# lcrekko/lq_mpc

Measured on AMD Instinct MI355X. Metric: MPC QP-steps/sec (batched systems) at n_x=4,n_u=2,N=10; 1/2/4/8 GPU, higher is better.
Workload: dtype f64

## Files before the change

lq_mpc_amd/csrc/lqmpc_r16_body.h:

```cpp
#pragma once
#include "lqmpc_wg_linalg.h"
#include "lqmpc_r16_setup.h"

namespace lqmpc {

using wg::ldsd;
using wg::ldsi;
using wg::rowb;
using wg::fmac_rowb;
using wg::fmac_rowb_self;
using wg::fmac_rowb4;
using wg::fmac_rowb_self4;
using wg::fmac_rowb_self2;
using wg::fmac_rowb_self3;
using wg::fmac_rowb_lanes4;
using wg::fmac_rowb_lanes4x2;
using wg::dpp_settle;

#ifdef LQMPC_R16_PROF
__device__ long long g_r16_prof[32];
#define RPROF(k) do { const long long now_ = clock64(); if (threadIdx.x == 0 && blockIdx.x == PROFBLK) g_r16_prof[k] += now_ - prof_t; if (k < 7) prof_ph[k] += now_ - prof_t; prof_t = clock64(); } while (0)
#define RPROF_START long long prof_t = clock64()
#define RPROF_ADD(k, v) do { if (threadIdx.x == 0) atomicAdd((unsigned long long *)&g_r16_prof[k], (unsigned long long)(v)); } while (0)
#ifndef PROFBLK
#define PROFBLK 0
#endif
#else
#define RPROF(k) do { } while (0)
#define RPROF_START do { } while (0)
#define RPROF_ADD(k, v) do { } while (0)
#endif

typedef unsigned long long mask_t;

template <int NX, int NU, int N, int LPI = 16, bool PACKED = false>
struct R16 {
    static constexpr int n = N * NU;
    static constexpr int RB = (n + LPI - 1) / LPI;
    static constexpr int IPW = 64 / LPI;
    static constexpr int CS = 4 * (((n + 1) / 2 + 3) / 4);
    static constexpr int LDW = n + 1;
    static constexpr int PK = PACKED ? n * (n + 1) / 2 : n * LDW;
    static constexpr int VEC = LPI * RB;
    static constexpr int oP = 0, oW = PK, oR = 2 * PK, oX = oR + VEC, oY = oX + VEC, oL = oY + VEC;
    static constexpr int oC = oL + CS / 2;
    static constexpr int CN0 = 3 * NX * NX + NU * NU + NX * NU;
    static constexpr int CN1 = (NX > NU ? NX : NU) * (2 * NX + 2 * NU);
    static constexpr int CN = CN0 > CN1 ? CN0 : CN1;
    static constexpr int SETUP = n * NX;
    static constexpr int oG = 0;
    static constexpr int END = oC + CN + (CN & 1);
    static constexpr int oD = (END > SETUP) ? END : SETUP;
    static constexpr int INST = oD + 2;
    static constexpr int MAXIT = 12;
    static_assert(LPI == 16 || LPI == 64, "a DPP row or the whole wavefront");
    static_assert((n + 1) / 2 <= CS && n <= 64, "the smaller side must fit the gathered system");
};


template <int LPI>
__device__ __forceinline__ mask_t iballot(bool c, int q)
{
    if constexpr (LPI == 16) return (__ballot(c) >> (16 * q)) & 0xFFFFull;
    else return __ballot(c);
}
template <int LPI>
__device__ __forceinline__ double ibcast(double x, int k)
{
    if constexpr (LPI == 16) return rowb(x, k);
    else return wg::rdlane(x, k);
}
template <int LPI>
__device__ __forceinline__ void ifmac(double &acc, double x, double y, int k)
{
    if constexpr (LPI == 16) fmac_rowb(acc, x, y, k);
    else acc = __builtin_fma(wg::rdlane(x, k), y, acc);
}
template <int LPI>
__device__ __forceinline__ void ifmac_self(double &acc, double y, int k)
{
    if constexpr (LPI == 16) fmac_rowb_self(acc, y, k);
    else acc = __builtin_fma(wg::rdlane(acc, k), y, acc);
}
template <int LPI>
__device__ __forceinline__ void ifmac4(double *acc, const double *x, double y, int k)
{
    if constexpr (LPI == 16) fmac_rowb4(acc[0], acc[1], acc[2], acc[3], x[0], x[1], x[2], x[3], y, k);
    else {
#pragma unroll
        for (int e = 0; e < 4; ++e) acc[e] = __builtin_fma(wg::rdlane(x[e], k), y, acc[e]);
    }
}
template <int LPI>
__device__ __forceinline__ void ifmac_self4(double *acc, double y, int k)
{
    if constexpr (LPI == 16) fmac_rowb_self4(acc[0], acc[1], acc[2], acc[3], y, k);
    else {
#pragma unroll
        for (int e = 0; e < 4; ++e) acc[e] = __builtin_fma(wg::rdlane(acc[e], k), y, acc[e]);
    }
}
template <int LPI, int K, int CS>
__device__ __forceinline__ void ifmac_self_tail(double (&S)[CS], double &rhs, double g)
{
    constexpr int r = K % 4;
    if constexpr (LPI == 16) {
        if constexpr (r == 0) fmac_rowb_self4(S[K + 1], S[K + 2], S[K + 3], rhs, g, K);
        else if constexpr (r == 1) fmac_rowb_self3(S[K + 1], S[K + 2], rhs, g, K);
        else if constexpr (r == 2) fmac_rowb_self2(S[K + 1], rhs, g, K);
        else fmac_rowb_self(rhs, g, K);
    } else {
#pragma unroll
        for (int j = K + 1; j < 4 * (K / 4) + 4; ++j) S[j] = __builtin_fma(wg::rdlane(S[j], K), g, S[j]);
        rhs = __builtin_fma(wg::rdlane(rhs, K), g, rhs);
    }
}
template <int LPI>
__device__ __forceinline__ void isettle(double &x)
{
    if constexpr (LPI == 16) dpp_settle(x);
}
__device__ __forceinline__ int rowb_i(int x, int c)
{
    switch (c) {
#define LQMPC_X(C) case C: return __builtin_amdgcn_update_dpp(0, x, 0x150 + C, 0xF, 0xF, true);
        LQMPC_ROWB_CASES(LQMPC_X)
#undef LQMPC_X
    }
    return x;
}
__device__ __forceinline__ unsigned row_or(unsigned x)
{
    x |= (unsigned)__builtin_amdgcn_update_dpp(0, (int)x, 0x128, 0xF, 0xF, false);
    x |= (unsigned)__builtin_amdgcn_update_dpp(0, (int)x, 0x124, 0xF, 0xF, false);
    x |= (unsigned)__builtin_amdgcn_update_dpp(0, (int)x, 0x122, 0xF, 0xF, false);
    x |= (unsigned)__builtin_amdgcn_update_dpp(0, (int)x, 0x121, 0xF, 0xF, false);
    return x;
}
__device__ __forceinline__ unsigned row_umax(unsigned x)
{
    x = max(x, (unsigned)__builtin_amdgcn_update_dpp(0, (int)x, 0x128, 0xF, 0xF, false));
    x = max(x, (unsigned)__builtin_amdgcn_update_dpp(0, (int)x, 0x124, 0xF, 0xF, false));
    x = max(x, (unsigned)__builtin_amdgcn_update_dpp(0, (int)x, 0x122, 0xF, 0xF, false));
    x = max(x, (unsigned)__builtin_amdgcn_update_dpp(0, (int)x, 0x121, 0xF, 0xF, false));
    return x;
}

template <int CNT, typename F>
__device__ __forceinline__ void static_for(F &&f) { sfor<0, CNT>(f); }

template <int NX, int NU, int N, int MODE, int LPI = 16, int OCC = 1>
__device__ __forceinline__ void r16_body(const KParams &p, double *lds_raw, long long slot0, long long slot_end)
{
    constexpr bool PACKED = (OCC == 2);
    using C = R16<NX, NU, N, LPI, PACKED>;
    constexpr int CS = C::CS;
    constexpr int n = C::n, RB = C::RB, LDW = C::LDW;
    constexpr int REC = NX * NX + NX * NU + NX;
    const int lane = threadIdx.x, q = lane / LPI, i = lane % LPI;
    ldsd *L = (ldsd *)lds_raw + q * C::INST;
    ldsd *Pp = L + C::oP, *Wp = L + C::oW, *rL = L + C::oR, *xL = L + C::oX, *yL = L + C::oY;
    ldsi *list = (ldsi *)(L + C::oL);
    const long long Bsz = p.Bsz;
    const long long b_raw = slot0 + q;
    const bool valid = b_raw < slot_end;
    const long long slot = valid ? b_raw : slot_end - 1;
    const long long b = p.perm ? (long long)p.perm[slot] : slot;
    const double *sh = p.sh;
    const mask_t nmask = (n == 64) ? ~0ull : ((1ull << n) - 1ull);

    int rw[RB], tri[RB];
    bool vrow[RB];
#pragma unroll
    for (int s = 0; s < RB; ++s) {
        rw[s] = i + LPI * s;
        tri[s] = rw[s] * (rw[s] + 1) / 2;
        vrow[s] = rw[s] < n;
    }

    auto ad = [&](int r, int tr, int j) -> int { if constexpr (PACKED) return (j <= r) ? tr + j : j * (j + 1) / 2 + r; else return r * LDW + j; };
    auto ad2 = [&](int a, int b2) -> int {
        if constexpr (PACKED) { const int hi = a > b2 ? a : b2, lo = a > b2 ? b2 : a; return hi * (hi + 1) / 2 + lo; }
        else return a * LDW + b2;
    };

    double G[RB][NX], vr[RB];
    constexpr bool LAZY_P = (LPI == 64);
    bool P_ready = !LAZY_P;
#ifdef LQMPC_NO_ROLL
    constexpr bool ROLL = false;
#else
    constexpr bool ROLL = LPI == 16 && N * ((NX + 3) / 4) <= 12 && MODE != MODE_MAXVN;
#endif
    unsigned cold32[2] = {0u, 0u};
    bool cold_armed = false;
#ifdef LQMPC_R16_PROF
    const long long prof_t0 = clock64();
    int prof_wit = 0, prof_slow = 0, prof_fast = 0;
    long long prof_slowt = 0;
    long long prof_ph[8] = {0, 0, 0, 0, 0, 0, 0, 0};
#endif
    {
        RPROF_START;
        long long bg = b;
        ldsd *Lg = L;
        if constexpr (LPI == 16) {
            const int gq = (lane >> 2) & 3;
            const long long sraw = slot0 + gq, sl = sraw < slot_end ? sraw : slot_end - 1;
            bg = p.perm ? (long long)p.perm[sl] : sl;
            Lg = (ldsd *)lds_raw + gq * C::INST;
        }
        r16_setup_mfma<NX, NU, N, LPI, PACKED, RB, ROLL>(setup_args(p), bg, Lg, L, C::oW, C::oG, C::oD, G, roll_args(p), cold32[0], cold32[1]);
        if constexpr (!LAZY_P) r16_build_P<NX, NU, N, LPI, PACKED>(setup_args(p), bg, Lg, C::oP, C::oD);
        RPROF(5);
        const bool has_lin = p.has_lin != 0;
#pragma unroll
        for (int s = 0; s < RB; ++s) vr[s] = 0.0;
        if (has_lin) {
            if (p.has_ref) {
                double qr[RB];
#pragma unroll
                for (int s = 0; s < RB; ++s) qr[s] = 0.0;
                double lam[NX], A2[NX][NX], B2[NX][NU];
#pragma unroll
                for (int a = 0; a < NX; ++a) {
                    lam[a] = 0.0;
#pragma unroll
                    for (int c = 0; c < NX; ++c) A2[a][c] = p.rec ? p.rec[b * REC + a * NX + c] : p.A[(long long)(a * NX + c) * Bsz + b];
#pragma unroll
                    for (int k = 0; k < NU; ++k) B2[a][k] = p.rec ? p.rec[b * REC + NX * NX + a * NU + k] : p.B[(long long)(a * NU + k) * Bsz + b];
                }
#pragma unroll 1
                for (int r = N - 1; r >= 0; --r) {
                    const int oQ = (r < N - 1) ? p.so.Q : p.so.P;
                    double l2[NX];
#pragma unroll
                    for (int a = 0; a < NX; ++a) {
                        double t = 0.0;
#pragma unroll
                        for (int c = 0; c < NX; ++c) t = __builtin_fma(sh[oQ + a * NX + c], -sh[p.so.xref + c * N + r], t);
#pragma unroll
                        for (int c = 0; c < NX; ++c) t = __builtin_fma(A2[c][a], lam[c], t);
                        l2[a] = t;
                    }
#pragma unroll
                    for (int a = 0; a < NX; ++a) lam[a] = l2[a];
#pragma unroll
                    for (int s = 0; s < RB; ++s) {
                        const int ui = rw[s] % NU;
                        double t = 0.0;
#pragma unroll
                        for (int k = 0; k < NU; ++k) {
                            double tk = 0.0;
#pragma unroll
                            for (int a = 0; a < NX; ++a) tk = __builtin_fma(B2[a][k], lam[a], tk);
#pragma unroll
                            for (int j = 0; j < NU; ++j) tk = __builtin_fma(-sh[p.so.R + k * NU + j], sh[p.so.uref + j * N + r], tk);
                            t = (ui == k) ? tk : t;
                        }
                        qr[s] = (vrow[s] && rw[s] / NU == r) ? 2.0 * t : qr[s];
                    }
                }
#pragma unroll
                for (int s = 0; s < RB; ++s) xL[rw[s]] = qr[s];
                __syncthreads();
#pragma unroll
                for (int s = 0; s < RB; ++s) {
                    double t = 0.0;
                    const int mr = vrow[s] ? rw[s] : 0, mt = vrow[s] ? tri[s] : 0;
#pragma unroll
                    for (int j = 0; j < n; ++j) t = __builtin_fma(Wp[ad(mr, mt, j)], xL[j], t);
                    vr[s] = -t;
                }
                __syncthreads();
            }
#pragma unroll
            for (int s = 0; s < RB; ++s) {
                const int k = rw[s] % NU;
                vr[s] = vrow[s] ? vr[s] - 0.5 * (sh[p.so.ub + k] + sh[p.so.lb + k]) : 0.0;
            }
        }
        if constexpr (LAZY_P && MODE != MODE_MAXVN) {
            mask_t out = 0;
#pragma unroll
            for (int s = 0; s < RB; ++s) {
                double acc = vr[s];
#pragma unroll
                for (int a = 0; a < NX; ++a) acc = __builtin_fma(G[s][a], p.rec ? p.rec[b * REC + NX * NX + NX * NU + a] : p.x0[(long long)a * Bsz + b], acc);
                const int k = rw[s] % NU;
                out |= iballot<LPI>(vrow[s] && !(fabs(acc) <= 0.5 * (sh[p.so.ub + k] - sh[p.so.lb + k])), q) << (LPI * s);
            }
            if (__ballot(2 * __popcll(out) > n) != 0ull) {
                r16_build_P<NX, NU, N, LPI, PACKED>(setup_args(p), bg, Lg, C::oP, C::oD);
                P_ready = true;
            }
        }
        RPROF(6);
    }
    RPROF_START;
    RPROF_ADD(13, clock64() - prof_t0);

    long long bq = b;
    asm volatile("" : "+v"(bq));
    double h[RB], ctr[RB];
#pragma unroll
    for (int s = 0; s < RB; ++s) {
        const int k = rw[s] % NU;
        h[s] = vrow[s] ? 0.5 * (sh[p.so.ub + k] - sh[p.so.lb + k]) : 1.0;
        ctr[s] = vrow[s] ? 0.5 * (sh[p.so.ub + k] + sh[p.so.lb + k]) : 0.0;
    }
    double Qm[NX][NX], Rm[NU][NU];
    ldsd *cQ = L + C::oC, *cR = cQ + NX * NX;
    if constexpr (MODE == MODE_ROLLOUT) {
    } else if constexpr (OCC == 2) {
        if (i == 0) {
#pragma unroll
            for (int a = 0; a < NX; ++a) {
#pragma unroll
                for (int c = 0; c < NX; ++c) {
                    cQ[a * NX + c] = sh[p.so.Q + a * NX + c];
                }
            }
#pragma unroll
            for (int k = 0; k < NU; ++k)
#pragma unroll
                for (int j = 0; j < NU; ++j) cR[k * NU + j] = sh[p.so.R + k * NU + j];
        }
        __syncthreads();
    } else {
#pragma unroll
        for (int a = 0; a < NX; ++a) {
#pragma unroll
            for (int c = 0; c < NX; ++c) Qm[a][c] = sh[p.so.Q + a * NX + c];
        }
#pragma unroll
        for (int k = 0; k < NU; ++k)
#pragma unroll
            for (int j = 0; j < NU; ++j) Rm[k][j] = sh[p.so.R + k * NU + j];
    }
    auto Qv = [&](int a, int c) -> double { if constexpr (OCC == 2) return cQ[a * NX + c]; else return Qm[a][c]; };
    auto Rv = [&](int k, int j) -> double { if constexpr (OCC == 2) return cR[k * NU + j]; else return Rm[k][j]; };
    const bool writer = valid && i == 0;
    mask_t pL = 0, pU = 0;
    int iters = 0, status = 0;
    auto qp = [&](const double (&x)[NX], double (&v)[RB]) {
        double vu[RB];
        mask_t cl = 0, cu = 0;
        bool bad = false;
#pragma unroll
        for (int s = 0; s < RB; ++s) {
            double acc = vr[s];
#pragma unroll
            for (int a = 0; a < NX; ++a) acc = __builtin_fma(G[s][a], x[a], acc);
            vu[s] = acc; v[s] = acc;
            cl |= iballot<LPI>(vrow[s] && acc < -h[s], q) << (LPI * s);
            cu |= iballot<LPI>(vrow[s] && acc > h[s], q) << (LPI * s);
            bad = bad || (vrow[s] && !(fabs(acc) < 1e300));
        }
        const bool rowbad = iballot<LPI>(bad, q) != 0;
        bool busy = ((cl | cu) != 0) && !rowbad;
        mask_t mL = 0, mU = 0;
        if (busy) {
            if (p.warm_start && (pL | pU) != 0) {
                const mask_t top = nmask & ~(nmask >> NU);
                mL = (pL >> NU) | (pL & top);
                mU = (pU >> NU) | (pU & top);
            } else if (ROLL && cold_armed && (cold32[0] | cold32[1]) != 0u) {
                mL = cold32[0]; mU = cold32[1];
            } else {
                mL = cl; mU = cu;
            }
        }
        cold_armed = false;
        bool failed = false;
        int it = 0;
        bool need_P = false;
#pragma unroll 1
        do {
        if (LAZY_P && need_P) {
            long long bg = bq;
            ldsd *Lg = L;
            if constexpr (LPI == 16) {
                const int gq = (lane >> 2) & 3;
                const long long sraw = slot0 + gq, sl = sraw < slot_end ? sraw : slot_end - 1;
                bg = p.perm ? (long long)p.perm[sl] : sl;
                Lg = (ldsd *)lds_raw + gq * C::INST;
            }
            r16_build_P<NX, NU, N, LPI, PACKED>(setup_args(p), bg, Lg, C::oP, C::oD);
            P_ready = true;
            need_P = false;
        }
        if (__ballot(busy) != 0ull) {
#pragma unroll 1
            for (; it < p.r16_maxit; ++it) {
#ifdef LQMPC_R16_PROF
                const long long prof_it0 = clock64();
#endif
                const mask_t mA = mL | mU;
                const int m = __popcll(mA);
                constexpr int DUAL_MAX = (LPI == 16 && n >= 16) ? (n / 2 + 2 < CS ? n / 2 + 2 : CS) : n / 2;
                const bool dual = m <= DUAL_MAX;
                const mask_t mC = busy ? (dual ? mA : (~mA & nmask)) : 0ull;
                const int c = __popcll(mC);
                int cw;
                if constexpr (LPI == 16)
                    cw = max(max(__builtin_amdgcn_readlane(c, 0), __builtin_amdgcn_readlane(c, 16)),
                             max(__builtin_amdgcn_readlane(c, 32), __builtin_amdgcn_readlane(c, 48)));
                else cw = __builtin_amdgcn_readfirstlane(c);
                const bool any_primal = __ballot(busy && !dual) != 0ull;
                if (LAZY_P && any_primal && !P_ready) { need_P = true; break; }
                if constexpr (LPI == 16) {
                    if (!any_primal) {
                        const unsigned mC32 = (unsigned)mC, mL32 = (unsigned)mL, mA32 = (unsigned)mA;
#pragma unroll
                        for (int s = 0; s < RB; ++s) {
                            const unsigned bit = 1u << rw[s];
                            const bool on = vrow[s] && (mC32 & bit);
                            const int rk = __popc(mC32 & (bit - 1u));
                            const double sg = (mL32 & bit) ? -1.0 : 1.0;
                            list[on ? rk : (C::oD - C::oL) * 2] = rw[s];
                            rL[on ? rk : C::oD - C::oR] = __builtin_fma(-sg, h[s], vu[s]);
                        }
                        __syncthreads();
                        const bool mine = i < c;
                        const int la = mine ? list[i] : 0;
                        double rhs = mine ? rL[i] : 0.0;
                        const int tla = PACKED ? la * (la + 1) / 2 : la * LDW;
                        auto widx = [&](int ra, int ta, int lb, int tlb) -> int {
                            if constexpr (PACKED) return max(ta, tlb) + min(ra, lb);
                            else return ta + lb;
                        };
                        double S[CS];
                        static_for<CS / 4>([&](auto bgc) {
                            constexpr int bg = decltype(bgc)::value;
#pragma unroll
                            for (int bb = 4 * bg; bb < 4 * bg + 4; ++bb) S[bb] = (bb == i) ? 1.0 : 0.0;
                            if (4 * bg < cw) {
                                static_for<4>([&](auto bc) {
                                    constexpr int bb = 4 * bg + decltype(bc)::value;
                                    const int lb = rowb_i(la, bb), tlb = PACKED ? rowb_i(tla, bb) : 0;
                                    const double val = Wp[widx(la, tla, lb, tlb)];
                                    S[bb] = mine ? val : S[bb];
                                });
                            }
                        });
                        bool ok = true;
                        static_for<CS>([&](auto kc) {
                            constexpr int k = decltype(kc)::value;
                            if (k < cw) {
                                isettle<LPI>(S[k]);
                                const double d = ibcast<LPI>(S[k], k);
                                ok = ok && (d > 0.0);
                                const double inv = frcp1(d);
                                const double g = (i == k) ? (inv - 1.0) : -S[k] * inv;
#pragma unroll
                                for (int jg = 0; jg < CS / 4; ++jg)
                                    if (4 * jg > k && 4 * jg < cw) ifmac_self4<LPI>(&S[4 * jg], g, k);
                                ifmac_self_tail<LPI, k>(S, rhs, g);
                            }
                        });
                        const bool rowfail = iballot<LPI>(!ok, q) != 0;
                        double tt[RB];
#pragma unroll
                        for (int s = 0; s < RB; ++s) tt[s] = 0.0;
                        const int trow[2] = {PACKED ? tri[0] : rw[0] * LDW, RB > 1 ? (PACKED ? tri[RB - 1] : rw[RB - 1] * LDW) : 0};
                        static_for<CS / 4>([&](auto kgc) {
                            constexpr int kg = decltype(kgc)::value;
                            if (4 * kg < cw) {
                                double wv[4][RB];
                                static_for<4>([&](auto kc) {
                                    constexpr int kk = decltype(kc)::value;
                                    const int lk = rowb_i(la, 4 * kg + kk), tlk = PACKED ? rowb_i(tla, 4 * kg + kk) : 0;
#pragma unroll
                                    for (int s = 0; s < RB; ++s) wv[kk][s] = Wp[vrow[s] ? widx(rw[s], trow[s], lk, tlk) : 0];
                                });
                                if constexpr (RB == 2) fmac_rowb_lanes4x2(tt[0], tt[1], rhs, wv[0][0], wv[0][1], wv[1][0], wv[1][1], wv[2][0], wv[2][1], wv[3][0], wv[3][1], 4 * kg);
                                else if constexpr (RB == 1) fmac_rowb_lanes4(tt[0], rhs, wv[0][0], wv[1][0], wv[2][0], wv[3][0], 4 * kg);
                                else {
                                    static_for<4>([&](auto kc) {
                                        constexpr int kk = decltype(kc)::value;
#pragma unroll
                                        for (int s = 0; s < RB; ++s) fmac_rowb(tt[s], rhs, wv[kk][s], 4 * kg + kk);
                                    });
                                }
                            }
                        });
                        const unsigned lhi = (unsigned)__double2hiint(rhs) & 0x7fffffffu;
                        const double tol = 1e-10 * __hiloint2double((int)row_umax(mine ? lhi : 0u), 0);
                        const bool isL = (mL32 >> la) & 1u;
                        const unsigned keepL = (mine && isL && rhs <= tol) ? (1u << la) : 0u;
                        const unsigned keepU = (mine && !isL && rhs >= -tol) ? (1u << la) : 0u;
                        unsigned nL32 = row_or(keepL), nU32 = row_or(keepU);
                        bool nf = false;
#pragma unroll
                        for (int s = 0; s < RB; ++s) {
                            const unsigned bit = 1u << rw[s];
                            const bool act = vrow[s] && (mA32 & bit);
                            const double sg = (mL32 & bit) ? -1.0 : 1.0;
                            const double nv = act ? sg * h[s] : vu[s] - tt[s];
                            v[s] = busy ? nv : v[s];
                            const bool fr = vrow[s] && !act;
                            nL32 |= (unsigned)(iballot<LPI>(fr && v[s] < -h[s] * (1.0 + 1e-12), q) << (LPI * s));
                            nU32 |= (unsigned)(iballot<LPI>(fr && v[s] > h[s] * (1.0 + 1e-12), q) << (LPI * s));
                            nf = nf || (vrow[s] && !(fabs(v[s]) < 1e300));
                        }
                        const bool rownf = iballot<LPI>(nf || (mine && !(fabs(rhs) < 1e300)), q) != 0;
#ifdef LQMPC_R16_PROF
                        prof_wit += 1; prof_fast += 1; prof_ph[7] += clock64() - prof_it0;
#endif
                        if (busy) {
                            iters += 1;
                            if (rowfail || rownf) { failed = true; busy = false; }
                            else if ((mask_t)nL32 == mL && (mask_t)nU32 == mU) busy = false;
                            else { mL = nL32; mU = nU32; }
                        }
                        __syncthreads();
                        if (__ballot(busy) == 0ull) break;
                        continue;
                    } else {
                        const unsigned mC32 = (unsigned)mC, mL32 = (unsigned)mL, mA32 = (unsigned)mA, mU32 = (unsigned)mU;
                        double rr[RB], z[RB];
#pragma unroll
                        for (int s = 0; s < RB; ++s) {
                            const unsigned bit = 1u << rw[s];
                            const bool act = vrow[s] && (mA32 & bit);
                            const double sg = (mL32 & bit) ? -1.0 : 1.0;
                            rr[s] = act ? __builtin_fma(-sg, h[s], vu[s]) : 0.0;
                            rL[rw[s]] = rr[s];
                            z[s] = 0.0;
                        }
                        __syncthreads();
#pragma unroll
                        for (int j = 0; j < n; ++j) {
                            const double rj = rL[j];
#pragma unroll
                            for (int s = 0; s < RB; ++s) z[s] = __builtin_fma(Pp[vrow[s] ? ad(rw[s], tri[s], j) : 0], rj, z[s]);
                        }
#pragma unroll
                        for (int s = 0; s < RB; ++s) {
                            const unsigned bit = 1u << rw[s];
                            const bool on = vrow[s] && (mC32 & bit);
                            const int rk = __popc(mC32 & (bit - 1u));
                            list[on ? rk : (C::oD - C::oL) * 2] = rw[s];
                            yL[on ? rk : C::oD - C::oY] = dual ? rr[s] : z[s];
                        }
                        __syncthreads();
                        const bool mine = i < c;
                        const int la = mine ? list[i] : 0;
                        double rhs = mine ? yL[i] : 0.0;
                        const int tla = PACKED ? la * (la + 1) / 2 : la * LDW;
                        const ldsd *Mx = dual ? Wp : Pp;
                        auto midx = [&](int ra, int ta, int lb, int tlb) -> int {
                            if constexpr (PACKED) return max(ta, tlb) + min(ra, lb);
                            else return ta + lb;
                        };
                        double S[CS];
                        static_for<CS / 4>([&](auto bgc) {
                            constexpr int bg = decltype(bgc)::value;
#pragma unroll
                            for (int bb = 4 * bg; bb < 4 * bg + 4; ++bb) S[bb] = (bb == i) ? 1.0 : 0.0;
                            if (4 * bg < cw) {
                                static_for<4>([&](auto bc) {
                                    constexpr int bb = 4 * bg + decltype(bc)::value;
                                    const int lb = rowb_i(la, bb), tlb = PACKED ? rowb_i(tla, bb) : 0;
                                    const double val = Mx[midx(la, tla, lb, tlb)];
                                    S[bb] = mine ? val : S[bb];
                                });
                            }
                        });
                        bool ok = true;
                        static_for<CS>([&](auto kc) {
                            constexpr int k = decltype(kc)::value;
                            if (k < cw) {
                                isettle<LPI>(S[k]);
                                const double d = ibcast<LPI>(S[k], k);
                                ok = ok && (d > 0.0);
                                const double inv = frcp1(d);
                                const double g = (i == k) ? (inv - 1.0) : -S[k] * inv;
#pragma unroll
                                for (int jg = 0; jg < CS / 4; ++jg)
                                    if (4 * jg > k && 4 * jg < cw) ifmac_self4<LPI>(&S[4 * jg], g, k);
                                ifmac_self_tail<LPI, k>(S, rhs, g);
                            }
                        });
                        const bool rowfail = iballot<LPI>(!ok, q) != 0;
                        if (mine) xL[la] = rhs;
                        double tt[RB];
#pragma unroll
                        for (int s = 0; s < RB; ++s) tt[s] = 0.0;
                        const int trow[2] = {PACKED ? tri[0] : rw[0] * LDW, RB > 1 ? (PACKED ? tri[RB - 1] : rw[RB - 1] * LDW) : 0};
                        static_for<CS / 4>([&](auto kgc) {
                            constexpr int kg = decltype(kgc)::value;
                            if (4 * kg < cw) {
                                double wv[4][RB];
                                static_for<4>([&](auto kc) {
                                    constexpr int kk = decltype(kc)::value;
                                    const int lk = rowb_i(la, 4 * kg + kk), tlk = PACKED ? rowb_i(tla, 4 * kg + kk) : 0;
#pragma unroll
                                    for (int s = 0; s < RB; ++s) wv[kk][s] = Mx[vrow[s] ? midx(rw[s], trow[s], lk, tlk) : 0];
                                });
                                if constexpr (RB == 2) fmac_rowb_lanes4x2(tt[0], tt[1], rhs, wv[0][0], wv[0][1], wv[1][0], wv[1][1], wv[2][0], wv[2][1], wv[3][0], wv[3][1], 4 * kg);
                                else if constexpr (RB == 1) fmac_rowb_lanes4(tt[0], rhs, wv[0][0], wv[1][0], wv[2][0], wv[3][0], 4 * kg);
                                else {
                                    static_for<4>([&](auto kc) {
                                        constexpr int kk = decltype(kc)::value;
#pragma unroll
                                        for (int s = 0; s < RB; ++s) fmac_rowb(tt[s], rhs, wv[kk][s], 4 * kg + kk);
                                    });
                                }
                            }
                        });
                        __syncthreads();
                        double gl[RB];
                        unsigned ghi = 0u;
#pragma unroll
                        for (int s = 0; s < RB; ++s) {
                            const unsigned bit = 1u << rw[s];
                            const bool act = vrow[s] && (mA32 & bit);
                            const double sg = (mL32 & bit) ? -1.0 : 1.0;
                            const double dl = xL[rw[s]];
                            const double nv = act ? sg * h[s] : (dual ? vu[s] - tt[s] : vu[s] + dl);
                            v[s] = busy ? nv : v[s];
                            gl[s] = (act && !dual) ? tt[s] - z[s] : 0.0;
                            ghi = max(ghi, (unsigned)__double2hiint(gl[s]) & 0x7fffffffu);
                        }
                        const unsigned lhi = (unsigned)__double2hiint(rhs) & 0x7fffffffu;
                        const double tol = 1e-10 * __hiloint2double((int)row_umax(dual ? (mine ? lhi : 0u) : ghi), 0);
                        const bool isL = (mL32 >> la) & 1u;
                        const unsigned keepL = (dual && mine && isL && rhs <= tol) ? (1u << la) : 0u;
                        const unsigned keepU = (dual && mine && !isL && rhs >= -tol) ? (1u << la) : 0u;
                        unsigned nL32 = row_or(keepL), nU32 = row_or(keepU);
                        bool nf = false;
#pragma unroll
                        for (int s = 0; s < RB; ++s) {
                            const unsigned bit = 1u << rw[s];
                            const bool act = vrow[s] && (mA32 & bit);
                            const bool fr = vrow[s] && !act;
                            const bool lo = (fr && v[s] < -h[s] * (1.0 + 1e-12)) || (act && !dual && (mL32 & bit) && gl[s] >= -tol);
                            const bool up = (fr && v[s] > h[s] * (1.0 + 1e-12)) || (act && !dual && (mU32 & bit) && gl[s] <= tol);
                            nL32 |= (unsigned)(iballot<LPI>(lo, q) << (LPI * s));
                            nU32 |= (unsigned)(iballot<LPI>(up, q) << (LPI * s));
                            nf = nf || (vrow[s] && !(fabs(v[s]) < 1e300));
                        }
                        const bool rownf = iballot<LPI>(nf || (mine && !(fabs(rhs) < 1e300)), q) != 0;
#ifdef LQMPC_R16_PROF
                        prof_wit += 1; prof_slow += 1; prof_slowt += clock64() - prof_it0;
#endif
                        if (busy) {
                            iters += 1;
                            if (rowfail || rownf) { failed = true; busy = false; }
                            else if ((mask_t)nL32 == mL && (mask_t)nU32 == mU) busy = false;
                            else { mL = nL32; mU = nU32; }
                        }
                        __syncthreads();
                        if (__ballot(busy) == 0ull) break;
                        continue;
                    }
                } else if (!any_primal) {
                    {
                        const mask_t bit = 1ull << rw[0];
                        const bool on = vrow[0] && (mC & bit);
                        const int rk = __popcll(mC & (bit - 1ull));
                        const double sg = (mL & bit) ? -1.0 : 1.0;
                        list[on ? rk : (C::oD - C::oL) * 2] = rw[0];
                        rL[on ? rk : C::oD - C::oR] = __builtin_fma(-sg, h[0], vu[0]);
                    }
                    __syncthreads();
                    const bool mine = i < c;
                    const int la = mine ? list[i] : 0;
                    double rhs = mine ? rL[i] : 0.0;
                    const int tla = PACKED ? la * (la + 1) / 2 : la * LDW;
                    auto widx = [&](int ra, int ta, int lb, int tlb) -> int {
                        if constexpr (PACKED) return max(ta, tlb) + min(ra, lb);
                        else return ta + lb;
                    };
                    double S[CS];
                    static_for<CS / 4>([&](auto bgc) {
                        constexpr int bg = decltype(bgc)::value;
#pragma unroll
                        for (int bb = 4 * bg; bb < 4 * bg + 4; ++bb) S[bb] = (bb == i) ? 1.0 : 0.0;
                        if (4 * bg < cw) {
                            static_for<4>([&](auto bc) {
                                constexpr int bb = 4 * bg + decltype(bc)::value;
                                const int lb = __builtin_amdgcn_readlane(la, bb), tlb = PACKED ? __builtin_amdgcn_readlane(tla, bb) : 0;
                                const double val = Wp[widx(la, tla, lb, tlb)];
                                S[bb] = mine ? val : S[bb];
                            });
                        }
                    });
                    bool ok = true;
                    static_for<CS>([&](auto kc) {
                        constexpr int k = decltype(kc)::value;
                        if (k < cw) {
                            const double d = ibcast<LPI>(S[k], k);
                            ok = ok && (d > 0.0);
                            const double inv = frcp1(d);
                            const double g = (i == k) ? (inv - 1.0) : -S[k] * inv;
#pragma unroll
                            for (int jg = 0; jg < CS / 4; ++jg)
                                if (4 * jg > k && 4 * jg < cw) ifmac_self4<LPI>(&S[4 * jg], g, k);
                            ifmac_self_tail<LPI, k>(S, rhs, g);
                        }
                    });
                    const bool rowfail = iballot<LPI>(!ok, q) != 0;
                    double tt = 0.0;
                    const int trow0 = PACKED ? tri[0] : rw[0] * LDW;
                    unsigned smax = 0u;
                    const unsigned lhi = (unsigned)__double2hiint(rhs) & 0x7fffffffu;
                    static_for<CS>([&](auto kc) {
                        constexpr int k = decltype(kc)::value;
                        if (k < cw) {
                            const int lk = __builtin_amdgcn_readlane(la, k), tlk = PACKED ? __builtin_amdgcn_readlane(tla, k) : 0;
                            const double wv = Wp[vrow[0] ? widx(rw[0], trow0, lk, tlk) : 0];
                            tt = __builtin_fma(wg::rdlane(rhs, k), wv, tt);
                            smax = max(smax, (unsigned)__builtin_amdgcn_readlane((int)lhi, k));
                        }
                    });
                    const double tol = 1e-10 * __hiloint2double((int)smax, 0);
                    const bool isL = (mL >> la) & 1ull;
                    const mask_t kL = __ballot(mine && isL && rhs <= tol), kU = __ballot(mine && !isL && rhs >= -tol);
                    mask_t nL = 0, nU = 0;
                    static_for<CS>([&](auto kc) {
                        constexpr int k = decltype(kc)::value;
                        if (k < cw) {
                            const int lk = __builtin_amdgcn_readlane(la, k);
                            nL |= ((kL >> k) & 1ull) << lk;
                            nU |= ((kU >> k) & 1ull) << lk;
                        }
                    });
                    {
                        const mask_t bit = 1ull << rw[0];
                        const bool act = vrow[0] && (mA & bit);
                        const double sg = (mL & bit) ? -1.0 : 1.0;
                        const double nv = act ? sg * h[0] : vu[0] - tt;
                        v[0] = busy ? nv : v[0];
                        const bool fr = vrow[0] && !act;
                        nL |= __ballot(fr && v[0] < -h[0] * (1.0 + 1e-12));
                        nU |= __ballot(fr && v[0] > h[0] * (1.0 + 1e-12));
                    }
                    const bool rownf = __ballot((vrow[0] && !(fabs(v[0]) < 1e300)) || (mine && !(fabs(rhs) < 1e300))) != 0ull;
#ifdef LQMPC_R16_PROF
                    prof_wit += 1; prof_fast += 1; prof_ph[7] += clock64() - prof_it0;
#endif
                    if (busy) {
                        iters += 1;
                        if (rowfail || rownf) { failed = true; busy = false; }
                        else if (nL == mL && nU == mU) busy = false;
                        else { mL = nL; mU = nU; }
                    }
                    __syncthreads();
                    if (__ballot(busy) == 0ull) break;
                    continue;
                }
#pragma unroll
                for (int s = 0; s < RB; ++s) {
                    const mask_t bit = 1ull << rw[s];
                    const double sg = (mL & bit) ? -1.0 : ((mU & bit) ? 1.0 : 0.0);
                    rL[rw[s]] = (sg != 0.0) ? vu[s] - sg * h[s] : 0.0;
                    xL[rw[s]] = 0.0;
                    if (vrow[s] && (mC & bit)) list[__popcll(mC & (bit - 1ull))] = rw[s];
                }
                __syncthreads();
                const ldsd *Mx = dual ? Wp : Pp;
                const int la = (i < c) ? list[i] : 0, tla = la * (la + 1) / 2;
                double S[CS], rhs;
                if constexpr (LPI == 16) {
                    const int tla2 = PACKED ? tla : la * LDW;
                    static_for<CS / 4>([&](auto bgc) {
                        constexpr int bg = decltype(bgc)::value;
#pragma unroll
                        for (int bb = 4 * bg; bb < 4 * bg + 4; ++bb) S[bb] = (bb == i) ? 1.0 : 0.0;
                        if (4 * bg < cw) {
                            static_for<4>([&](auto bc) {
                                constexpr int bb = 4 * bg + decltype(bc)::value;
                                const int lb = rowb_i(la, bb), tlb = PACKED ? rowb_i(tla2, bb) : 0;
                                int idx;
                                if constexpr (PACKED) idx = max(tla2, tlb) + min(la, lb); else idx = tla2 + lb;
                                const double val = Mx[idx];
                                S[bb] = (i < c) ? val : S[bb];
                            });
                        }
                    });
                } else {
#pragma unroll
                    for (int bg = 0; bg < CS / 4; ++bg) {
#pragma unroll
                        for (int bb = 4 * bg; bb < 4 * bg + 4; ++bb) S[bb] = (bb == i) ? 1.0 : 0.0;
                        if (4 * bg < cw) {
#pragma unroll
                            for (int bb = 4 * bg; bb < 4 * bg + 4; ++bb) {
                                const int lb = (bb < c) ? list[bb] : 0;
                                const double val = Mx[ad2(la, lb)];
                                if (i < c && bb < c) S[bb] = val;
                            }
                        }
                    }
                }
                rhs = (i < c && dual) ? rL[la] : 0.0;
                if (any_primal) {
                    double tp = 0.0;
#pragma unroll
                    for (int j = 0; j < n; ++j) tp = __builtin_fma(Pp[ad(la, tla, j)], rL[j], tp);
                    if (i < c && !dual) rhs = tp;
                }
                bool ok = true;
                static_for<CS>([&](auto kc) {
                    constexpr int k = decltype(kc)::value;
                    if (k < cw) {
                        isettle<LPI>(S[k]);
                        const double d = ibcast<LPI>(S[k], k);
                        ok = ok && (d > 0.0);
                        const double inv = frcp1(d);
                        const double g = (i == k) ? (inv - 1.0) : -S[k] * inv;
#pragma unroll
                        for (int jg = 0; jg < CS / 4; ++jg)
                            if (4 * jg > k && 4 * jg < cw) ifmac_self4<LPI>(&S[4 * jg], g, k);
                        ifmac_self_tail<LPI, k>(S, rhs, g);
                    }
                });
                const bool rowfail = iballot<LPI>(!ok, q) != 0;
                if (i < c) xL[la] = rhs;
                __syncthreads();
                double xs_[RB];
#pragma unroll
                for (int s = 0; s < RB; ++s) {
                    xs_[s] = xL[rw[s]];
                    yL[rw[s]] = dual ? xs_[s] : xs_[s] - rL[rw[s]];
                }
                __syncthreads();
                double tol = 0.0, gl[RB];
#pragma unroll
                for (int s = 0; s < RB; ++s) {
                    double tt = 0.0;
                    const int mr = vrow[s] ? rw[s] : 0, mt = vrow[s] ? tri[s] : 0;
#pragma unroll
                    for (int j = 0; j < n; ++j) tt = __builtin_fma(Mx[ad(mr, mt, j)], yL[j], tt);
                    const mask_t bit = 1ull << rw[s];
                    const bool act = vrow[s] && (mA & bit);
                    const double sg = (mL & bit) ? -1.0 : 1.0;
                    const double xs = xs_[s];
                    const double nv = act ? sg * h[s] : (dual ? vu[s] - tt : vu[s] + xs);
                    v[s] = busy ? nv : v[s];
                    gl[s] = act ? (dual ? -xs : tt) : 0.0;
                    tol = fmax(tol, fabs(gl[s]));
                }
                tol = fmax(tol, __shfl_xor(tol, 1)); tol = fmax(tol, __shfl_xor(tol, 2));
                tol = fmax(tol, __shfl_xor(tol, 4)); tol = fmax(tol, __shfl_xor(tol, 8));
                if (LPI == 64) { tol = fmax(tol, __shfl_xor(tol, 16)); tol = fmax(tol, __shfl_xor(tol, 32)); }
                tol *= 1e-10;
                mask_t nL = 0, nU = 0;
                bool nf = false;
#pragma unroll
                for (int s = 0; s < RB; ++s) {
                    const mask_t bit = 1ull << rw[s];
                    const bool act = vrow[s] && (mA & bit);
                    const bool lo = act ? ((mL & bit) && gl[s] >= -tol) : (vrow[s] && v[s] < -h[s] * (1.0 + 1e-12));
                    const bool up = act ? ((mU & bit) && gl[s] <= tol) : (vrow[s] && v[s] > h[s] * (1.0 + 1e-12));
                    nL |= iballot<LPI>(lo, q) << (LPI * s);
                    nU |= iballot<LPI>(up, q) << (LPI * s);
                    nf = nf || (vrow[s] && !(fabs(v[s]) < 1e300));
                }
                const bool rownf = iballot<LPI>(nf, q) != 0;
#ifdef LQMPC_R16_PROF
                prof_wit += 1; prof_slow += 1; prof_slowt += clock64() - prof_it0;
#endif
                if (busy) {
                    iters += 1;
                    if (rowfail || rownf) { failed = true; busy = false; }
                    else if (nL == mL && nU == mU) busy = false;
                    else { mL = nL; mU = nU; }
                }
                __syncthreads();
                if (__ballot(busy) == 0ull) break;
            }
        }
        } while (LAZY_P && need_P);
        if (busy) failed = true;
        if (failed || rowbad) {
            status = 3; pL = 0; pU = 0;
#pragma unroll
            for (int s = 0; s < RB; ++s) v[s] = fmin(fmax(vu[s], -h[s]), h[s]);
        } else {
            pL = mL; pU = mU;
        }
    };
    auto stage_input = [&](const double (&v)[RB], int st, double (&u)[NU]) {
#pragma unroll
        for (int k = 0; k < NU; ++k) {
            const int row = st * NU + k;
            const double uk = fmin(fmax(v[row / LPI], -h[row / LPI]), h[row / LPI]) + ctr[row / LPI];
            u[k] = ibcast<LPI>(uk, row % LPI);
        }
    };
    if (MODE != MODE_ROLLOUT) {
        double Am[NX][NX], Bmm[NX][NU], Pm[NX][NX];
        ldsd *cA = cR + NU * NU, *cB = cA + NX * NX, *cP = cB + NX * NU;
        if constexpr (OCC == 2) {
            if (i == 0) {
#pragma unroll
                for (int a = 0; a < NX; ++a) {
#pragma unroll
                    for (int c = 0; c < NX; ++c) {
                        cA[a * NX + c] = p.rec ? p.rec[bq * REC + a * NX + c] : p.A[(long long)(a * NX + c) * Bsz + bq];
                        cP[a * NX + c] = sh[p.so.P + a * NX + c];
                    }
#pragma unroll
                    for (int k = 0; k < NU; ++k) cB[a * NU + k] = p.rec ? p.rec[bq * REC + NX * NX + a * NU + k] : p.B[(long long)(a * NU + k) * Bsz + bq];
                }
            }
            __syncthreads();
        } else {
#pragma unroll
            for (int a = 0; a < NX; ++a) {
#pragma unroll
                for (int c = 0; c < NX; ++c) {
                    Am[a][c] = p.rec ? p.rec[bq * REC + a * NX + c] : p.A[(long long)(a * NX + c) * Bsz + bq];
                    Pm[a][c] = sh[p.so.P + a * NX + c];
                }
#pragma unroll
                for (int k = 0; k < NU; ++k) Bmm[a][k] = p.rec ? p.rec[bq * REC + NX * NX + a * NU + k] : p.B[(long long)(a * NU + k) * Bsz + bq];
            }
        }
        auto Av = [&](int a, int c) -> double { if constexpr (OCC == 2) return cA[a * NX + c]; else return Am[a][c]; };
        auto Bv = [&](int a, int k) -> double { if constexpr (OCC == 2) return cB[a * NU + k]; else return Bmm[a][k]; };
        auto Pv = [&](int a, int c) -> double { if constexpr (OCC == 2) return cP[a * NX + c]; else return Pm[a][c]; };
        auto value_fn = [&](const double (&x0v)[NX], const double (&v)[RB]) -> double {
            double xs[NX], c = 0.0;
#pragma unroll
            for (int a = 0; a < NX; ++a) xs[a] = x0v[a];
#pragma unroll
            for (int a = 0; a < NX; ++a)
#pragma unroll
                for (int cc = 0; cc < NX; ++cc) c = __builtin_fma(xs[a] * Qv(a, cc), xs[cc], c);
#pragma unroll
            for (int s = 0; s < RB; ++s) xL[rw[s]] = vrow[s] ? fmin(fmax(v[s], -h[s]), h[s]) + ctr[s] : 0.0;
            __syncthreads();
#pragma unroll 1
            for (int st = 0; st < N; ++st) {
                double u[NU], xn[NX];
#pragma unroll
                for (int k = 0; k < NU; ++k) u[k] = xL[st * NU + k];
#pragma unroll
                for (int a = 0; a < NX; ++a) {
                    double acc = 0.0;
#pragma unroll
                    for (int cc = 0; cc < NX; ++cc) acc = __builtin_fma(Av(a, cc), xs[cc], acc);
#pragma unroll
                    for (int k = 0; k < NU; ++k) acc = __builtin_fma(Bv(a, k), u[k], acc);
                    xn[a] = acc;
                }
#pragma unroll
                for (int a = 0; a < NX; ++a) { xs[a] = xn[a]; if (p.has_ref) xn[a] -= sh[p.so.xref + a * N + st]; }
#pragma unroll
                for (int a = 0; a < NX; ++a)
#pragma unroll
                    for (int cc = 0; cc < NX; ++cc) c = __builtin_fma(xn[a] * ((st == N - 1) ? Pv(a, cc) : Qv(a, cc)), xn[cc], c);
                if (p.has_ref) {
#pragma unroll
                    for (int k = 0; k < NU; ++k) u[k] -= sh[p.so.uref + k * N + st];
                }
#pragma unroll
                for (int k = 0; k < NU; ++k)
#pragma unroll
                    for (int j = 0; j < NU; ++j) c = __builtin_fma(u[k] * Rv(k, j), u[j], c);
            }
            __syncthreads();
            return c;
        };
        if (MODE == MODE_SOLVE) {
            double x[NX], v[RB], u[NU];
#pragma unroll
            for (int a = 0; a < NX; ++a) x[a] = p.rec ? p.rec[bq * REC + NX * NX + NX * NU + a] : p.x0[(long long)a * Bsz + bq];
            cold_armed = ROLL;
            qp(x, v);
            const double vn = value_fn(x, v);
            stage_input(v, 0, u);
            if (writer) {
                p.VN[b] = vn;
#pragma unroll
                for (int k = 0; k < NU; ++k) p.u0[(long long)k * Bsz + bq] = u[k];
            }
        } else {
            double best = -1e308;
            for (int kk = 0; kk < p.K; ++kk) {
                double x[NX], v[RB];
#pragma unroll
                for (int a = 0; a < NX; ++a) x[a] = sh[p.so.x0s + a * p.K + kk];
                pL = 0; pU = 0;
                qp(x, v);
                const double vn = value_fn(x, v);
                best = (vn > best || vn != vn) ? vn : best;
            }
            if (writer) p.MV[b] = best;
        }
    }
    if (MODE == MODE_ROLLOUT || MODE == MODE_SWEEP) {
        pL = 0; pU = 0;
        double x[NX];
#pragma unroll
        for (int a = 0; a < NX; ++a) x[a] = p.rec ? p.rec[bq * REC + NX * NX + NX * NU + a] : p.x0[(long long)a * Bsz + bq];
        int ia = i < NX ? i : 0, ik = i < NU ? i : 0;
        asm volatile("" : "+v"(ia), "+v"(ik));
        double Qr_[NX], Ar_[NX], Br_[NU], Rr_[NU];
#pragma unroll
        for (int c = 0; c < NX; ++c) {
            Qr_[c] = sh[p.so.Q + ia * NX + c];
            Ar_[c] = p.true_per_instance ? p.At[(long long)(ia * NX + c) * Bsz + bq] : sh[p.so.At + ia * NX + c];
        }
#pragma unroll
        for (int k = 0; k < NU; ++k) {
            Br_[k] = p.true_per_instance ? p.Bt[(long long)(ia * NU + k) * Bsz + bq] : sh[p.so.Bt + ia * NU + k];
            Rr_[k] = sh[p.so.R + ik * NU + k];
        }
        constexpr bool ROWS_IN_LDS = OCC == 2 && LPI == 64 && 2 * NX + 2 * NU > 12;
        constexpr int RW = 2 * NX + 2 * NU;
        static_assert((NX > NU ? NX : NU) * RW <= C::CN + (C::CN & 1), "the per-lane rows fit the constants region");
        ldsd *myc = L + C::oC + ((i < NX || i < NU) ? i : 0) * RW;
        if constexpr (ROWS_IN_LDS) {
            __syncthreads();
            if (i < NX || i < NU) {
#pragma unroll
                for (int c = 0; c < NX; ++c) { myc[c] = Ar_[c]; myc[NX + NU + c] = Qr_[c]; }
#pragma unroll
                for (int k = 0; k < NU; ++k) { myc[NX + k] = Br_[k]; myc[2 * NX + NU + k] = Rr_[k]; }
            }
            __syncthreads();
        }
        auto Ar = [&](int c) -> double { if constexpr (ROWS_IN_LDS) return myc[c]; else return Ar_[c]; };
        auto Br = [&](int k) -> double { if constexpr (ROWS_IN_LDS) return myc[NX + k]; else return Br_[k]; };
        auto Qr = [&](int c) -> double { if constexpr (ROWS_IN_LDS) return myc[NX + NU + c]; else return Qr_[c]; };
        auto Rr = [&](int k) -> double { if constexpr (ROWS_IN_LDS) return myc[2 * NX + NU + k]; else return Rr_[k]; };
        double costx, costu = 0.0;
        {
            double xm = x[0], qx = 0.0;
#pragma unroll
            for (int a = 1; a < NX; ++a) xm = (i == a) ? x[a] : xm;
#pragma unroll
            for (int c = 0; c < NX; ++c) qx = __builtin_fma(Qr(c), x[c], qx);
            costx = xm * qx;
        }
        if (p.X && writer) {
#pragma unroll
            for (int a = 0; a < NX; ++a) p.X[((long long)a * (p.T + 1)) * Bsz + bq] = x[a];
        }
#ifdef LQMPC_R16_PROF
        long long prof_ts = 0, prof_acc[5] = {0, 0, 0, 0, 0};
#endif
        for (int t = 0; t < p.T; ++t) {
            double v[RB], u[NU], xn[NX];
#ifdef LQMPC_R16_PROF
            if (t == 1) { RPROF_ADD(27, clock64() - prof_ts); RPROF_ADD(28, prof_wit); RPROF_ADD(29, prof_slow); }
            if (t > 0) {
                const long long d_ = clock64() - prof_ts;
                if (prof_wit) { prof_acc[1] += d_; prof_acc[3] += 1; prof_acc[4] += prof_wit; } else { prof_acc[0] += d_; prof_acc[2] += 1; }
            }
            prof_ts = clock64();
            prof_wit = 0;
#endif
            bool inside = false;
            {
                bool out = false;
#pragma unroll
                for (int s = 0; s < RB; ++s) {
                    double acc = vr[s];
#pragma unroll
                    for (int a = 0; a < NX; ++a) acc = __builtin_fma(G[s][a], x[a], acc);
                    v[s] = acc;
                    out = out || (vrow[s] && !(fabs(acc) <= h[s]));
                }
                inside = __ballot(out) == 0ull;
            }
            cold_armed = ROLL && t == 0;
            if (inside) { pL = 0; pU = 0; }
            else qp(x, v);
            const double um = fmin(fmax(v[0], -h[0]), h[0]) + ctr[0];
            stage_input(v, 0, u);
            double xm = 0.0, qx = 0.0, ru = 0.0;
#pragma unroll
            for (int c = 0; c < NX; ++c) xm = __builtin_fma(Ar(c), x[c], xm);
#pragma unroll
            for (int k = 0; k < NU; ++k) xm = __builtin_fma(Br(k), u[k], xm);
#pragma unroll
            for (int a = 0; a < NX; ++a) xn[a] = ibcast<LPI>(xm, a);
#pragma unroll
            for (int a = 0; a < NX; ++a) x[a] = xn[a];
#pragma unroll
            for (int c = 0; c < NX; ++c) qx = __builtin_fma(Qr(c), xn[c], qx);
            costx = __builtin_fma(xm, qx, costx);
#pragma unroll
            for (int j = 0; j < NU; ++j) ru = __builtin_fma(Rr(j), u[j], ru);
            costu = __builtin_fma(um, ru, costu);
            if (writer) {
                if (p.X) {
#pragma unroll
                    for (int a = 0; a < NX; ++a) p.X[((long long)a * (p.T + 1) + t + 1) * Bsz + bq] = xn[a];
                }
                if (p.U) {
#pragma unroll
                    for (int k = 0; k < NU; ++k) p.U[((long long)k * p.T + t) * Bsz + bq] = u[k];
                }
            }
        }
        double cost = 0.0;
#pragma unroll
        for (int a = 0; a < NX; ++a) cost += ibcast<LPI>(costx, a);
#pragma unroll
        for (int k = 0; k < NU; ++k) cost += ibcast<LPI>(costu, k);
        RPROF(7);
#ifdef LQMPC_R16_PROF
        for (int k_ = 0; k_ < 5; ++k_) RPROF_ADD(8 + k_, prof_acc[k_]);
#endif
        RPROF_ADD(14, clock64() - prof_t0); RPROF_ADD(15, 1); RPROF_ADD(16, prof_slow); RPROF_ADD(30, prof_slow > 0 ? 1 : 0);
#ifdef LQMPC_R16_PROF
        for (int k_ = 0; k_ < 8; ++k_) RPROF_ADD(17 + k_, prof_ph[k_]);
        RPROF_ADD(25, prof_slowt); RPROF_ADD(26, prof_fast);
#endif
        if (writer) p.JT[b] = cost;
    }
    if (writer) {
        if (p.status) p.status[b] = status;
        if (p.iters) p.iters[b] = iters;
        if (status == 3 && p.fail_list) p.fail_list[atomicAdd(p.fail_count, 1)] = (int)b;
    }
}

}
```

Baseline: 7.044 billion.

## Replace LDS round-trips with lane broadcasts in active-set correction step

The z = P·r product now broadcasts residual values across the row's lanes with DPP/row broadcast helpers instead of writing them to LDS and hitting a barrier. It splits the work into two accumulators to shorten the FMA dependency chain. The write of the solved rhs to xL, and the barrier after it, are replaced by a __shfl gather indexed by each row's rank in the constrained set. This removes two workgroup barriers and LDS traffic per inner iteration, but relies on the row values living within the LPI-lane group, so the mapping must be correct.

```diff
diff --git a/lq_mpc_amd/csrc/lqmpc_r16_body.h b/lq_mpc_amd/csrc/lqmpc_r16_body.h
--- a/lq_mpc_amd/csrc/lqmpc_r16_body.h
+++ b/lq_mpc_amd/csrc/lqmpc_r16_body.h
@@ -519,23 +519,40 @@
                         continue;
                     } else {
                         const unsigned mC32 = (unsigned)mC, mL32 = (unsigned)mL, mA32 = (unsigned)mA, mU32 = (unsigned)mU;
-                        double rr[RB], z[RB];
+                        double rr[RB], z[RB], z2[RB];
 #pragma unroll
                         for (int s = 0; s < RB; ++s) {
                             const unsigned bit = 1u << rw[s];
                             const bool act = vrow[s] && (mA32 & bit);
                             const double sg = (mL32 & bit) ? -1.0 : 1.0;
                             rr[s] = act ? __builtin_fma(-sg, h[s], vu[s]) : 0.0;
-                            rL[rw[s]] = rr[s];
-                            z[s] = 0.0;
-                        }
-                        __syncthreads();
-#pragma unroll
-                        for (int j = 0; j < n; ++j) {
-                            const double rj = rL[j];
-#pragma unroll
-                            for (int s = 0; s < RB; ++s) z[s] = __builtin_fma(Pp[vrow[s] ? ad(rw[s], tri[s], j) : 0], rj, z[s]);
-                        }
+                            z[s] = 0.0; z2[s] = 0.0;
+                        }
+                        static_for<(n + 3) / 4>([&](auto jgc) {
+                            constexpr int jg = decltype(jgc)::value, j0 = 4 * jg, sj = j0 / LPI, c0 = j0 % LPI;
+                            {
+                                double pv[4][RB];
+                                static_for<4>([&](auto kc) {
+                                    constexpr int kk = decltype(kc)::value, j = j0 + kk;
+#pragma unroll
+                                    for (int s = 0; s < RB; ++s) pv[kk][s] = Pp[(vrow[s] && j < n) ? ad(rw[s], tri[s], j) : 0];
+                                });
+                                auto acc = [&](double (&za)[RB]) {
+                                    if constexpr (RB == 2) fmac_rowb_lanes4x2(za[0], za[1], rr[sj], pv[0][0], pv[0][1], pv[1][0], pv[1][1], pv[2][0], pv[2][1], pv[3][0], pv[3][1], c0);
+                                    else if constexpr (RB == 1) fmac_rowb_lanes4(za[0], rr[sj], pv[0][0], pv[1][0], pv[2][0], pv[3][0], c0);
+                                    else {
+                                        static_for<4>([&](auto kc) {
+                                            constexpr int kk = decltype(kc)::value;
+#pragma unroll
+                                            for (int s = 0; s < RB; ++s) fmac_rowb(za[s], rr[sj], pv[kk][s], c0 + kk);
+                                        });
+                                    }
+                                };
+                                if constexpr (jg % 2 == 0) acc(z); else acc(z2);
+                            }
+                        });
+#pragma unroll
+                        for (int s = 0; s < RB; ++s) z[s] += z2[s];
 #pragma unroll
                         for (int s = 0; s < RB; ++s) {
                             const unsigned bit = 1u << rw[s];
@@ -584,7 +601,12 @@
                             }
                         });
                         const bool rowfail = iballot<LPI>(!ok, q) != 0;
-                        if (mine) xL[la] = rhs;
+                        double dl[RB];
+#pragma unroll
+                        for (int s = 0; s < RB; ++s) {
+                            const int rk = __popc(mC32 & ((1u << rw[s]) - 1u)) & (LPI - 1);
+                            dl[s] = __shfl(rhs, (lane & ~(LPI - 1)) | rk);
+                        }
                         double tt[RB];
 #pragma unroll
                         for (int s = 0; s < RB; ++s) tt[s] = 0.0;
@@ -610,7 +632,6 @@
                                 }
                             }
                         });
-                        __syncthreads();
                         double gl[RB];
                         unsigned ghi = 0u;
 #pragma unroll
@@ -618,8 +639,7 @@
                             const unsigned bit = 1u << rw[s];
                             const bool act = vrow[s] && (mA32 & bit);
                             const double sg = (mL32 & bit) ? -1.0 : 1.0;
-                            const double dl = xL[rw[s]];
-                            const double nv = act ? sg * h[s] : (dual ? vu[s] - tt[s] : vu[s] + dl);
+                            const double nv = act ? sg * h[s] : (dual ? vu[s] - tt[s] : vu[s] + dl[s]);
                             v[s] = busy ? nv : v[s];
                             gl[s] = (act && !dual) ? tt[s] - z[s] : 0.0;
                             ghi = max(ghi, (unsigned)__double2hiint(gl[s]) & 0x7fffffffu);
```

After: 7.035 billion, median of 2. Within noise of the previous version (-0.1%).
